# guptakhil/show-tell

Measured on AMD Instinct MI355X. Metric: training images/sec (ResNet101+GRU, emb=512, bs=128) at 1/2/4/8 MI355X, higher is better.
Workload: dtype bf16; 1 GPU; BASELINE configs[1]: ResNet-101 (train-mode BN, frozen) + 5-layer GRU decoder, E=H=512, V=10000, fwd+bwd+SGD step, synthetic COCO-shaped batch; batch_per_gpu=128, global_batch=128, image=3x224x224, parallelism=dp1

## Files before the change

### include/showtell_hip.h

```cpp
#ifndef SHOWTELL_HIP_H
#define SHOWTELL_HIP_H

#include <stddef.h>
#include <stdint.h>

#ifdef __cplusplus
extern "C" {
#endif

#define ST_F32 0
#define ST_BF16 1

#define ST_CELL_GRU 0
#define ST_CELL_LSTM 1

const char* st_last_error(void);
int st_version(void);

typedef struct {
  const void* x;
  const void* w;
  void* y;
  const float* bias;
  const float* scale;
// ... 24 lines not shown
} st_conv3x3_img_desc;
int st_conv3x3_img_supported(int H, int W, int C, int N);
int st_conv3x3_img(const st_conv3x3_img_desc* d, void* stream);
int st_conv3x3_s2_supported(int C, int N);
int st_conv3x3_s2(const st_conv3x3_img_desc* d, void* stream);
typedef struct {
  const void* x; const void* w_frag; void* y; const void* residual;
  float* stats; int stats_replicas;
  const float* scale; const float* shift; int relu;
  const float* in_stats; const float* in_gamma; const float* in_beta; float in_count; float in_eps; int in_stats_replicas;
  int B, Hin, Win, C, N, stride;
} st_conv1x1_wreg_desc;
int st_conv1x1_wreg_supported(int C, int N);
int st_conv1x1_wreg(const st_conv1x1_wreg_desc* d, void* stream);
int st_conv1x1_kstream_supported(int C, int N);
int st_conv1x1_kstream(const st_conv1x1_wreg_desc* d, void* stream);
typedef struct {
  const void* raw; const void* identity; void* x_out; const void* w_frag; void* y;
  float* stats; int stats_replicas;
  const float* f_stats; const float* f_gamma; const float* f_beta; float f_count; float f_eps; int f_stats_replicas;
  long rows; int C, N;
  const float* id_stats; const float* id_gamma; const float* id_beta; int id_stats_replicas;
} st_conv1x1_kfuse_desc;
int st_conv1x1_kfuse_supported(int C, int N);
int st_conv1x1_kfuse(const st_conv1x1_kfuse_desc* d, void* stream);
#ifdef ST_EXPERIMENTAL
int st_conv1x1_kfuse8(const st_conv1x1_kfuse_desc* d, void* stream);
#endif
typedef struct {
  const void* raw2; const void* w3_frag; const void* identity; void* x_out; const void* w1_frag; void* y;
  float* stats; int stats_replicas;
  const float* bn2_stats; const float* bn2_gamma; const float* bn2_beta; int bn2_replicas;
  const float* bn3_stats; const float* bn3_gamma; const float* bn3_beta; int bn3_replicas;
  const float* id_stats; const float* id_gamma; const float* id_beta; int id_replicas;
  float count; float eps;
  long rows; int C1, C2, N;
} st_conv_b2b_desc;
int st_conv_b2b_supported(int C1, int C2, int N);
int st_conv_b2b(const st_conv_b2b_desc* d, void* stream);
typedef struct {
  const void* x2; const void* w3_frag; const void* identity; void* x_out; const void* w1_frag; void* y;
  float* stats; int stats_replicas;
  const float* bn2_stats; const float* bn2_gamma; const float* bn2_beta; int bn2_replicas;
  const float* bn3_stats; const float* bn3_gamma; const float* bn3_beta; int bn3_replicas;
  float count; float eps;
  const float* scale3; const float* shift3; const float* scale1; const float* shift1; int relu1;
  long rows; int C1, C2, N;
  const float* id_stats; const float* id_gamma; const float* id_beta; int id_replicas;
} st_conv_c3c1_desc;
int st_conv_c3c1_supported(int C1, int C2, int N);
int st_conv_c3c1(const st_conv_c3c1_desc* d, void* stream);
int st_conv1x1_astat_supported(int C, int N);
int st_conv1x1_astat(const st_conv1x1_wreg_desc* d, void* stream);

int st_pack_conv_weight_frag(const float* w, void* out, int Cout, int Cin, int KH, int KW, int ntw, void* stream);

int st_tune(int reserved, int kc, int w8);
int st_prof_enable(int on);
int st_debug_stamps(unsigned long long* buf);
int st_prof_collect(double* ms, double* flops, long* launches);

typedef struct {
  const void* x; void* y; const void* res;
  const float* stats;  const float* gamma; const float* beta;
  const float* running_mean; const float* running_var;
  const float* res_stats; const float* res_gamma; const float* res_beta;
  const float* res_running_mean; const float* res_running_var;
  int res_bn;
  int dtype; long rows; int C; float count; float eps; int relu;
  int stats_replicas, res_stats_replicas;
} st_bn_act_desc;

int st_bn_act(const st_bn_act_desc* d, void* stream);

int st_bn_update_running(const float* stats, float* running_mean, float* running_var,
                         int C, float count, float momentum, void* stream);

int st_nchw_to_nhwc(const float* x, void* y, int dtype, int B, int C, int H, int W, int Cpad, void* stream);
int st_nchw_to_s2d16(const float* x, void* y, int dtype, int B, int H, int W, void* stream);
int st_stem_weight_s2d(const void* w, void* out, int dtype, int Cpad, void* stream);
int st_nhwc_to_ncp_f32(const void* x, float* y, int dtype, int B, int HW, int C, void* stream);
int st_maxpool3x3s2(const void* x, void* y, int dtype, int B, int H, int W, int C, void* stream);
int st_maxpool3x3s2_bn(const void* x, void* y, int dtype, int B, int H, int W, int C,
                       const float* stats, const float* gamma, const float* beta,
                       const float* running_mean, const float* running_var, float count, float eps, void* stream);
typedef struct {
  const void* x_s2d; const void* w_frag; void* y;
  float* stats; int stats_replicas;
  const float* gamma;
  const float* scale; const float* shift;
  int B, H, W;
} st_stem_conv_pool_desc;
int st_stem_conv_pool(const st_stem_conv_pool_desc* d, void* stream);
int st_stem_weight_frag(const void* w_s2d, void* out, void* stream);
int st_stem_weight_frag_packed(const void* w_packed, int Cpad, void* out, void* stream);
int st_global_avgpool(const void* x, void* y, int dtype, int out_dtype, int B, int HW, int C, void* stream);

typedef struct st_image_batch_desc {
  const uint8_t* src;
  int64_t src_bytes;
  const int64_t* offset;
  const int32_t* height;
  const int32_t* width;
  const int32_t* flip;
  int batch;
  int max_height, max_width;
// ... 161 lines not shown
```

### show-tell_amd/_lib.py

```python
import ctypes as C
import os

_HERE = os.path.dirname(os.path.abspath(__file__))
LIB_PATH = os.path.join(_HERE, "lib", "libshowtell_hip.so")

ST_F32, ST_BF16 = 0, 1
ST_CELL_GRU, ST_CELL_LSTM = 0, 1

c_p, c_i, c_f, c_l = C.c_void_p, C.c_int, C.c_float, C.c_long


class ConvDesc(C.Structure):
    _fields_ = [("x", c_p), ("w", c_p), ("y", c_p), ("bias", c_p), ("scale", c_p), ("shift", c_p),
                ("residual", c_p), ("stats", c_p), ("dtype", c_i), ("out_dtype", c_i),
                ("B", c_i), ("Hin", c_i), ("Win", c_i), ("Cin", c_i), ("Ho", c_i), ("Wo", c_i), ("N", c_i),
                ("KH", c_i), ("KW", c_i), ("stride", c_i), ("pad", c_i),
                ("ldx", c_i), ("ldw", c_i), ("ldy", c_i), ("relu", c_i), ("accumulate", c_i), ("Cin_logical", c_i), ("k_order", c_i), ("stats_replicas", c_i),
                ("in_stats", c_p), ("in_gamma", c_p), ("in_beta", c_p), ("in_count", c_f), ("in_eps", c_f), ("split_k", c_i)]


class Conv3x3ImgDesc(C.Structure):
    _fields_ = [("x", c_p), ("w_frag", c_p), ("y", c_p), ("stats", c_p), ("stats_replicas", c_i), ("scale", c_p), ("shift", c_p),
                ("relu", c_i), ("in_stats", c_p), ("in_gamma", c_p), ("in_beta", c_p), ("in_count", c_f), ("in_eps", c_f),
                ("B", c_i), ("H", c_i), ("W", c_i), ("C", c_i), ("N", c_i), ("in_stats_replicas", c_i)]
# ... 49 lines not shown


class RnnParams(C.Structure):
    _fields_ = [("cell", c_i), ("dtype", c_i), ("L", c_i), ("in0", c_i), ("H", c_i), ("V", c_i), ("E", c_i),
                ("emb", c_p), ("w_ih", c_p * ST_MAX_LAYERS), ("w_hh", c_p * ST_MAX_LAYERS),
                ("b_ih", c_p * ST_MAX_LAYERS), ("b_hh", c_p * ST_MAX_LAYERS), ("w_lin", c_p), ("b_lin", c_p)]


class RnnGrads(C.Structure):
    _fields_ = [("emb", c_p), ("w_ih", c_p * ST_MAX_LAYERS), ("w_hh", c_p * ST_MAX_LAYERS),
                ("b_ih", c_p * ST_MAX_LAYERS), ("b_hh", c_p * ST_MAX_LAYERS), ("w_lin", c_p), ("b_lin", c_p)]


class AttnParams(C.Structure):
    _fields_ = [("rnn", RnnParams), ("F", c_i), ("A", c_i), ("P", c_i),
                ("w_enc", c_p), ("b_enc", c_p), ("w_dec", c_p), ("b_dec", c_p), ("w_full", c_p), ("b_full", c_p),
                ("w_init_h", c_p), ("b_init_h", c_p), ("w_init_c", c_p), ("b_init_c", c_p), ("w_embed", c_p), ("b_embed", c_p)]


class AttnGrads(C.Structure):
    _fields_ = [("rnn", RnnGrads)] + [(n, c_p) for n in ("w_enc", "b_enc", "w_dec", "b_dec", "w_full", "b_full", "w_init_h", "b_init_h",
                                                        "w_init_c", "b_init_c", "w_embed", "b_embed")]


class PackedSeq(C.Structure):
    _fields_ = [("B", c_i), ("T", c_i), ("ntok", c_i), ("Tcap", c_i), ("batch_sizes_host", C.POINTER(c_i)),
                ("rows_b", c_p), ("rows_t", c_p), ("prev_row", c_p), ("caption", c_p)]


class ImageBatchDesc(C.Structure):
    _fields_ = [("src", c_p), ("src_bytes", C.c_int64), ("offset", c_p), ("height", c_p), ("width", c_p), ("flip", c_p), ("batch", c_i),
                ("max_height", c_i), ("max_width", c_i), ("out_h", c_i), ("out_w", c_i), ("lut", c_p), ("tmp", c_p),
                ("out", c_p), ("out_u8", c_p)]


_SIGS = {
    "st_version": ([], c_i),
    "st_image_transform": ([C.POINTER(ImageBatchDesc), c_p], c_i),
    "st_conv": ([C.POINTER(ConvDesc), c_p], c_i),
    "st_conv_batch": ([C.POINTER(ConvDesc), c_i, c_p], c_i),
    "st_conv3x3_img_supported": ([c_i, c_i, c_i, c_i], c_i),
    "st_conv3x3_img": ([C.POINTER(Conv3x3ImgDesc), c_p], c_i),
    "st_conv3x3_s2_supported": ([c_i, c_i], c_i),
    "st_conv3x3_s2": ([C.POINTER(Conv3x3ImgDesc), c_p], c_i),
    "st_conv1x1_wreg_supported": ([c_i, c_i], c_i),
    "st_conv1x1_wreg": ([C.POINTER(Conv1x1WregDesc), c_p], c_i),
    "st_conv1x1_kfuse": ([C.POINTER(Conv1x1KfuseDesc), c_p], c_i),
    "st_conv1x1_kfuse_supported": ([c_i, c_i], c_i),
    "st_conv1x1_kfuse8": ([C.POINTER(Conv1x1KfuseDesc), c_p], c_i),
    "st_conv_b2b": ([C.POINTER(ConvB2bDesc), c_p], c_i),
    "st_conv_b2b_supported": ([c_i, c_i, c_i], c_i),
    "st_conv1x1_astat_supported": ([c_i, c_i], c_i),
    "st_conv1x1_astat": ([C.POINTER(Conv1x1WregDesc), c_p], c_i),
    "st_conv1x1_kstream_supported": ([c_i, c_i], c_i),
    "st_conv1x1_kstream": ([C.POINTER(Conv1x1WregDesc), c_p], c_i),
    "st_pack_conv_weight_frag": ([c_p, c_p, c_i, c_i, c_i, c_i, c_i, c_p], c_i),
    "st_tune": ([c_i, c_i, c_i], c_i),
    "st_prof_enable": ([c_i], c_i),
    "st_debug_stamps": ([c_p], c_i),
    "st_prof_collect": ([C.POINTER(C.c_double), C.POINTER(C.c_double), C.POINTER(c_l)], c_i),
    "st_bn_act": ([C.POINTER(BnActDesc), c_p], c_i),
    "st_bn_update_running": ([c_p, c_p, c_p, c_i, c_f, c_f, c_p], c_i),
    "st_nchw_to_nhwc": ([c_p, c_p, c_i, c_i, c_i, c_i, c_i, c_i, c_p], c_i),
    "st_nchw_to_s2d16": ([c_p, c_p, c_i, c_i, c_i, c_i, c_p], c_i),
    "st_stem_weight_s2d": ([c_p, c_p, c_i, c_i, c_p], c_i),
    "st_stem_weight_frag": ([c_p, c_p, c_p], c_i),
    "st_stem_weight_frag_packed": ([c_p, c_i, c_p, c_p], c_i),
    "st_stem_conv_pool": ([C.POINTER(StemConvPoolDesc), c_p], c_i),
    "st_nhwc_to_ncp_f32": ([c_p, c_p, c_i, c_i, c_i, c_i, c_p], c_i),
    "st_maxpool3x3s2": ([c_p, c_p, c_i, c_i, c_i, c_i, c_i, c_p], c_i),
    "st_maxpool3x3s2_bn": ([c_p, c_p, c_i, c_i, c_i, c_i, c_i, c_p, c_p, c_p, c_p, c_p, c_f, c_f, c_p], c_i),
    "st_global_avgpool": ([c_p, c_p, c_i, c_i, c_i, c_i, c_i, c_p], c_i),
    "st_cast": ([c_p, c_p, c_i, c_i, c_l, c_p], c_i),
    "st_transpose": ([c_p, c_p, c_i, c_i, c_i, c_i, c_i, c_p], c_i),
    "st_transpose_colsum": ([c_p, c_p, c_p, c_i, c_i, c_i, c_i, c_i, c_p], c_i),
    "st_transpose_batch": ([c_p, c_p, c_p, c_i, c_i, c_i, c_i, c_i, c_i, c_p, c_p, c_p], c_i),
    "st_pack_conv_weight": ([c_p, c_p, c_i, c_i, c_i, c_i, c_i, c_i, c_i, c_p], c_i),
    "st_cast2d": ([c_p, c_p, c_i, c_i, c_i, c_i, c_i, c_i, c_p], c_i),
    "st_rnn_vocab_ld": ([c_i], c_i),
    "st_rnn_workspace_bytes": ([C.POINTER(RnnParams), C.POINTER(PackedSeq)], C.c_size_t),
    "st_rnn_forward": ([C.POINTER(RnnParams), C.POINTER(PackedSeq), c_p, c_p, c_p, C.c_size_t, c_p, c_i, c_i, c_p, c_i, c_p], c_i),
    "st_rnn_fused_loss_supported": ([C.POINTER(RnnParams)], c_i),
    "st_rnn_fused_loss_bytes": ([C.POINTER(RnnParams), C.POINTER(PackedSeq)], C.c_size_t),
    "st_rnn_fused_loss": ([C.POINTER(RnnParams), C.POINTER(PackedSeq), c_p, C.c_size_t, c_p, c_p, C.c_size_t, c_p, c_p], c_i),
    "st_rnn_fused_dlogits": ([C.POINTER(RnnParams), C.POINTER(PackedSeq), c_p, C.c_size_t, c_p, c_p, c_p, c_p, c_i, c_p], c_i),
    "st_rnn_backward": ([C.POINTER(RnnParams), C.POINTER(RnnGrads), C.POINTER(PackedSeq), c_p, c_p, c_i, c_p, c_p, C.c_size_t,
                         c_p, c_p, c_p], c_i),
    "st_rnn_greedy_workspace_bytes": ([C.POINTER(RnnParams), c_i], C.c_size_t),
    "st_rnn_greedy": ([C.POINTER(RnnParams), c_p, c_i, c_i, c_p, C.c_size_t, c_p, c_p, c_p], c_i),
    "st_rnn_greedy_last_route": ([], c_i),
    "st_rnn_step": ([C.POINTER(RnnParams), c_p, c_i, c_p, c_p, c_p, c_p, c_p, c_i, c_p], c_i),
    "st_embedding_rows": ([c_p, c_p, c_p, c_i, c_i, c_i, c_i, c_i, c_p], c_i),
    "st_gather_state": ([c_p, c_p, c_p, c_i, c_i, c_i, c_i, c_i, c_p], c_i),
    "st_softmax_topk": ([c_p, c_i, c_i, c_i, c_i, c_p, c_p, c_i, c_p], c_i),
    "st_beam_select": ([c_p, c_p, c_p, c_p, c_p, c_i, c_i, c_i, c_l, c_p, c_p, c_p, c_p, c_p, c_p], c_i),
    "st_sample_rows": ([c_p, c_i, c_i, c_i, c_p, c_i, c_f, c_i, c_l, c_p, c_p, c_p, c_i, c_i, c_p, c_p], c_i),
    "st_rnn_sample_workspace_bytes": ([C.POINTER(RnnParams), c_i], C.c_size_t),
    "st_rnn_sample": ([C.POINTER(RnnParams), c_p, c_i, c_i, c_p, c_f, c_i, c_l, c_p, C.c_size_t, c_p, c_p, c_p], c_i),
    "st_attn_workspace_bytes": ([c_p, c_p], C.c_size_t),
    "st_attn_forward": ([c_p, c_p, c_p, c_p, c_p, C.c_size_t, c_p, c_i, c_i, c_p, c_i, c_p], c_i),
    "st_attn_backward": ([c_p, c_p, c_p, c_p, c_p, c_i, c_p, c_p, c_f, c_p, c_p, C.c_size_t, c_p], c_i),
    "st_attn_reg_loss": ([c_p, c_i, c_i, c_i, c_f, c_p, c_p], c_i),
    "st_attn_greedy_workspace_bytes": ([c_p, c_i], C.c_size_t),
    "st_attn_greedy": ([c_p, c_p, c_i, c_i, c_l, c_p, C.c_size_t, c_p, c_p], c_i),
    "st_attn_greedy_alphas": ([c_p, c_p, c_i, c_i, c_l, c_p, C.c_size_t, c_p, c_p, c_p], c_i),
    "st_attn_sample_workspace_bytes": ([c_p, c_i], C.c_size_t),
# ... 66 lines not shown
```

### show-tell_amd/csrc/resnet.cpp

```cpp
#include "common.h"
#include <vector>
#include <map>
#include <mutex>
#include <new>
#include <string>
#include <string.h>
#include <stdlib.h>

struct ConvL { int cin, cout, k, stride, pad; size_t woff; size_t bnoff; int korder; size_t woff_frag; int ntw; };
struct BlockL { int c1, c2, c3, ds; int stride; };
static inline bool use_astat(const ConvL& c) {
  if (c.k != 1) return false;
  if (c.stride == 1) return (c.cin == 256 && c.cout == 1024) || (c.cin == 512 && c.cout == 2048);
  return c.stride == 2 && ((c.cin == 256 && c.cout == 512) || (c.cin == 512 && c.cout == 1024));
}

struct BnTable { int n; int end[160]; float count[160]; int soff[160]; int rep[160]; };
struct PendingUpdate { BnTable tab; const float* stats; };

struct st_resnet {
  int version, dtype, bottleneck, cpad0;
  std::vector<ConvL> convs;
  std::vector<BlockL> blocks;
  size_t wtotal = 0, bntotal = 0;
// ... 116 lines not shown
        b.c2 = add(planes[li], planes[li], 3, s, 1);
        b.c3 = add(planes[li], planes[li] * 4, 1, 1, 0);
      } else {
        b.c1 = add(inpl, planes[li], 3, s, 1);
        b.c2 = add(planes[li], planes[li], 3, 1, 1);
      }
      if (bi == 0 && (s != 1 || inpl != planes[li] * exp)) b.ds = add(inpl, planes[li] * exp, 1, s, 0);
      inpl = planes[li] * exp;
      r->blocks.push_back(b);
    }
  r->feat_dim = inpl;
  ST_CHECK(r->convs.size() <= 160, "st_resnet_create: too many layers");
  *out = r;
  return 0;
}

extern "C" void st_resnet_destroy(st_resnet* r) { delete r; }
extern "C" int st_resnet_num_convs(const st_resnet* r) { return r ? (int)r->convs.size() : -1; }
extern "C" int st_resnet_feat_dim(const st_resnet* r) { return r ? r->feat_dim : -1; }
extern "C" size_t st_resnet_weight_elems(const st_resnet* r) { return r ? r->wtotal : 0; }
extern "C" size_t st_resnet_bn_channels(const st_resnet* r) { return r ? r->bntotal : 0; }

extern "C" int st_resnet_conv_info(const st_resnet* r, int i, int* cin, int* cout, int* k, int* stride, int* pad,
                                   int* cin_padded, size_t* weight_offset, size_t* bn_offset, int* k_order,
                                   size_t* frag_weight_offset, int* frag_ntw) {
  ST_CHECK(r && i >= 0 && i < (int)r->convs.size(), "st_resnet_conv_info: bad index %d", i);
  const ConvL& c = r->convs[i];
  if (cin) *cin = c.cin;
  if (cout) *cout = c.cout;
  if (k) *k = c.k;
  if (stride) *stride = c.stride;
  if (pad) *pad = c.pad;
  if (cin_padded) *cin_padded = c.cin == 3 ? r->cpad0 : c.cin;
  if (weight_offset) *weight_offset = c.woff;
  if (bn_offset) *bn_offset = c.bnoff;
  if (k_order) *k_order = c.korder;
  if (frag_weight_offset) *frag_weight_offset = c.woff_frag;
  if (frag_ntw) *frag_ntw = c.ntw;
  return 0;
}

extern "C" int st_resnet_set_taps(st_resnet* r, void* buf, size_t bytes) {
  ST_CHECK(r && (buf || bytes == 0), "st_resnet_set_taps: null pointer");
  std::lock_guard<std::mutex> lk(r->mu);
  r->taps = buf; r->taps_bytes = buf ? bytes : 0;
  return 0;
}

namespace {
FILE* layer_log() {
  static FILE* f = [] { const char* e = getenv("ST_LAYER_LOG"); return e && *e ? fopen(e, "w") : nullptr; }();
  return f;
}
struct Layout { size_t in_bytes, s2dw_bytes, stem_bytes, wide_bytes, narrow_bytes, stats_bytes, fold_bytes, total; };
inline bool stem_s2d(int H, int W) { return H % 2 == 0 && W % 2 == 0; }
Layout make_layout(const st_resnet* r, int B, int H, int W) {
  const size_t es = st_dtype_size(r->dtype);
  Layout p;
  p.in_bytes = align256((size_t)B * H * W * r->cpad0 * es);
  if (stem_s2d(H, W)) { const size_t b2 = align256((size_t)B * (H / 2 + 3) * (W / 2 + 3) * 16 * es); if (b2 > p.in_bytes) p.in_bytes = b2; }
  p.s2dw_bytes = align256((size_t)64 * 256 * es);
  const int h1 = conv_out(H, 7, 2, 3), w1 = conv_out(W, 7, 2, 3);
  p.stem_bytes = align256((size_t)B * h1 * w1 * 64 * es);
  const int h2 = conv_out(h1, 3, 2, 1), w2 = conv_out(w1, 3, 2, 1);
  const size_t wide_c = r->bottleneck ? 256 : 64;
  p.wide_bytes = align256((size_t)B * h2 * w2 * wide_c * es);
  p.narrow_bytes = align256((size_t)B * h2 * w2 * 128 * es);
  p.stats_bytes = align256((2 * r->bntotal + (size_t)kStatsRepFloats * r->convs.size()) * sizeof(float));
  p.fold_bytes = align256(2 * r->bntotal * sizeof(float));
  p.total = p.in_bytes + p.s2dw_bytes + p.stem_bytes + 3 * p.wide_bytes + 2 * p.narrow_bytes + p.stats_bytes + p.fold_bytes;
  return p;
}

enum Route {
  R_IGEMM, R_IMG, R_S2, R_WREG, R_ASTAT, R_KSTREAM,
  R_KFUSE, R_B2B, R_B2B0, R_C3C1,
  R_STEM, R_STEM_POOL, R_MAXPOOL,
  R_BN_ACT, R_REDUCE, R_TAP
};
enum Slot { S_NONE = -1, S_IN, S_STEM, S_WIDE, S_NARROW = S_WIDE + 3, S_COUNT = S_NARROW + 2 };

struct Launch {
  Route route;
  int ci;
  int hin, win;
  int x, y, res, xout;
  int relu;
  int in_ci;
  int pc;
  int id_ci;
  int rep_out, rep_in;
};
constexpr int kMaxLaunches = 768;
struct FwdPlan { int n; bool s2d; int h, w, out; BnTable tab; Launch l[kMaxLaunches]; };

int plan_forward(const st_resnet* r, int B, int H, int W, bool train, FwdPlan& p) {
  const int nconv = (int)r->convs.size(), nblk = (int)r->blocks.size();
  ST_CHECK(nconv <= 160 && 8 + 14 * nblk <= kMaxLaunches, "st_resnet_forward: too many layers");
  const bool bf16 = r->dtype == ST_BF16;
  BnTable& tab = p.tab;
  tab.n = nconv;
  for (int i = 0; i < nconv; ++i) { tab.end[i] = (int)(r->convs[i].bnoff + r->convs[i].cout); tab.count[i] = 1.f; tab.soff[i] = 0; tab.rep[i] = 1; }
  int hin[160], win[160], hout[160], wout[160];
  Route rt[160];
  auto geo = [&](int ci, int h, int w, bool res) {
    const ConvL& c = r->convs[ci];
    hin[ci] = h; win[ci] = w;
    hout[ci] = conv_out(h, c.k, c.stride, c.pad); wout[ci] = conv_out(w, c.k, c.stride, c.pad);
    tab.count[ci] = (float)((long)B * hout[ci] * wout[ci]);
    rt[ci] = R_IGEMM;
    if (!bf16 || c.ntw == 0) return;
    if (c.k == 1 && (!res || (c.stride == 1 && c.cin <= 512))) rt[ci] = use_astat(c) ? R_ASTAT : c.cin > 512 ? R_KSTREAM : R_WREG;
    else if (c.k == 3 && c.stride == 1 && !res && st_conv3x3_img_supported(h, w, c.cin, c.cout) == c.ntw) rt[ci] = R_IMG;
    else if (c.k == 3 && c.stride == 2 && !res && st_conv3x3_s2_supported(c.cin, c.cout) == c.ntw && (long)B * h * w * c.cin * 2 < (1L << 31))
      rt[ci] = R_S2;
  };
  geo(0, H, W, false);
  rt[0] = R_STEM;
  int h = conv_out(hout[0], 3, 2, 1), w = conv_out(wout[0], 3, 2, 1);
  for (const BlockL& b : r->blocks) {
    geo(b.c1, h, w, false);
    if (b.ds >= 0) geo(b.ds, h, w, false);
    if (r->bottleneck) { geo(b.c2, hout[b.c1], wout[b.c1], false); geo(b.c3, hout[b.c2], wout[b.c2], !train); }
// ... 159 lines not shown
    case R_BN_ACT:
      fam = "bn_act"; what = l.res != S_NONE ? "bn + identity + relu" : "bn + relu"; cin = c.cout; k = stride = hin = win = 0;
      by = rows * c.cout * (l.res != S_NONE ? 3.0 : 2.0) * es; break;
    case R_REDUCE:
      fam = "bn_reduce_replicas"; what = "statistics replicas -> replica 0"; cin = c.cout; k = stride = hin = win = 0; break;
    default: return 0;
  }
  return snprintf(buf, n, "%s,%s,%d,%d,%d,%d,%d,%d,%.0f,%.0f,%d,%d\n", fam, what, cin, cout, k, stride, hin, win, fl, by, l.rep_out, l.rep_in);
}
}

extern "C" size_t st_resnet_workspace_bytes(const st_resnet* r, int B, int H, int W) {
  if (!r || B <= 0 || H < 32 || W < 32) return 0;
  return make_layout(r, B, H, W).total;
}

extern "C" int st_resnet_plan(const st_resnet* r, int B, int H, int W, int train, char* buf, size_t bytes) {
  if (!r || B <= 0 || H < 32 || W < 32) { st_set_error("st_resnet_plan: bad arguments"); return -1; }
  FwdPlan p;
  if (plan_forward(r, B, H, W, train != 0, p)) return -1;
  std::string text;
  char line[256];
  for (int i = 0; i < p.n; ++i) text.append(line, format_launch(r, B, p.l[i], line, sizeof(line)));
  if (buf && bytes > text.size()) memcpy(buf, text.c_str(), text.size() + 1);
  return (int)text.size();
}

extern "C" int st_resnet_forward(const st_resnet* r, const float* images_nchw, int B, int H, int W,
                                 const void* weights, const float* bn_gamma, const float* bn_beta,
                                 float* bn_running_mean, float* bn_running_var,
                                 int train, float momentum, float eps,
                                 void* workspace, size_t workspace_bytes,
                                 void* feat_nhwc_out, void* pooled_out, int pooled_dtype, float* ncp_out,
                                 void* stream) {
  ST_CHECK(r && images_nchw && weights && bn_gamma && bn_beta && bn_running_mean && bn_running_var && workspace,
           "st_resnet_forward: null pointer");
  ST_CHECK(B > 0 && H >= 32 && W >= 32, "st_resnet_forward: bad input size %dx%dx%d", B, H, W);
  const Layout lay = make_layout(r, B, H, W);
  ST_CHECK(workspace_bytes >= lay.total, "st_resnet_forward: workspace too small (%zu < %zu)", workspace_bytes, lay.total);
  FwdPlan p;
  if (plan_forward(r, B, H, W, train != 0, p)) return 1;
  const BnTable& tab = p.tab;
  hipStream_t st = reinterpret_cast<hipStream_t>(stream);
  const int dt = r->dtype;
  const size_t es = st_dtype_size(dt);
  char* ws = reinterpret_cast<char*>(workspace);
  char* slot[S_COUNT];
  slot[S_IN] = ws; ws += lay.in_bytes;
  char* s2dw = ws; ws += lay.s2dw_bytes;
  slot[S_STEM] = ws; ws += lay.stem_bytes;
  for (int i = 0; i < 3; ++i) { slot[S_WIDE + i] = ws; ws += lay.wide_bytes; }
  for (int i = 0; i < 2; ++i) { slot[S_NARROW + i] = ws; ws += lay.narrow_bytes; }
  float* stats = reinterpret_cast<float*>(ws); ws += lay.stats_bytes;
  float* fold = reinterpret_cast<float*>(ws);
  const int total = (int)r->bntotal;
  float* fscale = fold; float* fshift = fold + total;

  if (train) {
    if (hipMemsetAsync(stats, 0, lay.stats_bytes, st) != hipSuccess) { st_set_error("memset failed"); return 1; }
  } else {
    hipLaunchKernelGGL(bn_fold_kernel, dim3((total + 255) / 256), dim3(256), 0, st, bn_gamma, bn_beta, bn_running_mean,
                       bn_running_var, fscale, fshift, total, eps);
    ST_LAUNCH_CHECK();
  }
  if (p.s2d) {
    if (st_nchw_to_s2d16(images_nchw, slot[S_IN], dt, B, H, W, stream)) return 1;
  } else if (st_nchw_to_nhwc(images_nchw, slot[S_IN], dt, B, 3, H, W, r->cpad0, stream)) return 1;

  auto S = [&](int s) -> void* { return s == S_NONE ? nullptr : slot[s]; };
  auto wts = [&](size_t off) { return reinterpret_cast<const char*>(weights) + off * es; };
  struct BnRef { const float* stats; const float* gamma; const float* beta; int rep; };
  auto bn = [&](int ci) { const ConvL& c = r->convs[ci]; return BnRef{stats + tab.soff[ci], bn_gamma + c.bnoff, bn_beta + c.bnoff, tab.rep[ci]}; };
  auto set_in = [&](auto& d, const Launch& l) {
    if (l.in_ci < 0) return;
    const BnRef b = bn(l.in_ci);
    d.in_stats = b.stats; d.in_gamma = b.gamma; d.in_beta = b.beta; d.in_count = tab.count[l.in_ci]; d.in_eps = eps;
  };
  auto set_out = [&](auto& d, const Launch& l) {
    const ConvL& c = r->convs[l.ci];
    if (train) { d.stats = stats + tab.soff[l.ci]; d.stats_replicas = l.rep_out; }
    else { d.scale = fscale + c.bnoff; d.shift = fshift + c.bnoff; d.relu = l.relu; }
  };
  auto set_fused = [&](auto& k, const Launch& l) {
    const BnRef b2 = bn(l.in_ci), b3 = bn(l.pc);
    k.bn2_stats = b2.stats; k.bn2_gamma = b2.gamma; k.bn2_beta = b2.beta; k.bn2_replicas = b2.rep;
    k.bn3_stats = b3.stats; k.bn3_gamma = b3.gamma; k.bn3_beta = b3.beta; k.bn3_replicas = b3.rep;
    if (l.id_ci >= 0) { const BnRef i = bn(l.id_ci); k.id_stats = i.stats; k.id_gamma = i.gamma; k.id_beta = i.beta; k.id_replicas = i.rep; }
    k.count = tab.count[l.pc]; k.eps = eps;
  };
  size_t taps_used = 0;
  auto run = [&](const Launch& l) -> int {
    const ConvL& c = r->convs[l.ci];
    const long rows = (long)B * l.hin * l.win;
    switch (l.route) {
      case R_STEM: case R_IGEMM: {
        st_conv_desc d{};
        const int cin_p = c.cin == 3 ? r->cpad0 : c.cin;
        d.x = S(l.x); d.w = wts(c.woff); d.y = S(l.y); d.residual = S(l.res);
        d.dtype = dt; d.out_dtype = dt;
        d.B = B; d.Hin = l.hin; d.Win = l.win; d.Cin = cin_p;
        d.Ho = conv_out(l.hin, c.k, c.stride, c.pad); d.Wo = conv_out(l.win, c.k, c.stride, c.pad);
        d.N = c.cout; d.KH = c.k; d.KW = c.k; d.stride = c.stride; d.pad = c.pad;
        d.ldx = cin_p; d.ldw = c.k * c.k * cin_p; d.ldy = c.cout; d.Cin_logical = c.cin; d.k_order = c.korder;
        if (l.route == R_STEM && p.s2d) {
          if (st_stem_weight_s2d(wts(c.woff), s2dw, dt, r->cpad0, stream)) return 1;
          d.w = s2dw; d.Hin = l.hin / 2 + 3; d.Win = l.win / 2 + 3; d.Cin = 64; d.ldx = 16; d.KH = 4; d.KW = 1; d.stride = 1; d.pad = 0;
          d.ldw = 256; d.Cin_logical = 36;
        }
        set_in(d, l); set_out(d, l);
        return st_conv(&d, stream);
      }
      case R_IMG: case R_S2: {
        st_conv3x3_img_desc g{};
        g.x = S(l.x); g.w_frag = wts(c.woff_frag); g.y = S(l.y);
        g.B = B; g.H = l.hin; g.W = l.win; g.C = c.cin; g.N = c.cout; g.in_stats_replicas = l.rep_in;
        set_in(g, l); set_out(g, l);
        return l.route == R_IMG ? st_conv3x3_img(&g, stream) : st_conv3x3_s2(&g, stream);
      }
      case R_WREG: case R_ASTAT: case R_KSTREAM: {
        st_conv1x1_wreg_desc g{};
        g.x = S(l.x); g.w_frag = wts(c.woff_frag); g.y = S(l.y); g.residual = S(l.res);
        g.B = B; g.Hin = l.hin; g.Win = l.win; g.C = c.cin; g.N = c.cout; g.stride = c.stride; g.in_stats_replicas = l.rep_in;
        set_in(g, l); set_out(g, l);
        if (l.route == R_WREG) return st_conv1x1_wreg(&g, stream);
        if (l.route == R_ASTAT) return st_conv1x1_astat(&g, stream);
        ST_CHECK(!g.in_stats, "st_resnet_forward: the long-K pointwise kernel has no input transform");
        return st_conv1x1_kstream(&g, stream);
      }
      case R_KFUSE: {
        st_conv1x1_kfuse_desc k{};
        const BnRef f = bn(l.pc);
        k.raw = S(l.x); k.identity = S(l.res); k.x_out = S(l.xout); k.w_frag = wts(c.woff_frag); k.y = S(l.y);
        k.stats = stats + tab.soff[l.ci]; k.stats_replicas = l.rep_out;
        k.f_stats = f.stats; k.f_gamma = f.gamma; k.f_beta = f.beta; k.f_count = tab.count[l.pc]; k.f_eps = eps; k.f_stats_replicas = f.rep;
        k.rows = rows; k.C = c.cin; k.N = c.cout;
        if (l.id_ci >= 0) { const BnRef i = bn(l.id_ci); k.id_stats = i.stats; k.id_gamma = i.gamma; k.id_beta = i.beta; k.id_stats_replicas = i.rep; }
        return st_conv1x1_kfuse(&k, stream);
      }
      case R_B2B: case R_B2B0: {
        const ConvL& c3 = r->convs[l.pc];
        st_conv_b2b_desc k{};
        k.raw2 = S(l.x); k.w3_frag = wts(c3.woff_frag); k.identity = S(l.res); k.x_out = S(l.xout);
        set_fused(k, l);
        k.rows = rows; k.C1 = c3.cin; k.C2 = c3.cout;
        if (l.route == R_B2B) {
          k.w1_frag = wts(c.woff_frag); k.y = S(l.y); k.stats = stats + tab.soff[l.ci]; k.stats_replicas = l.rep_out; k.N = c.cout;
        }
        return st_conv_b2b(&k, stream);
      }
      case R_C3C1: {
        const ConvL& c3 = r->convs[l.pc];
        st_conv_c3c1_desc k{};
        k.x2 = S(l.x); k.w3_frag = wts(c3.woff_frag); k.identity = S(l.res); k.x_out = S(l.xout); k.w1_frag = wts(c.woff_frag); k.y = S(l.y);
        if (train) {
          k.stats = stats + tab.soff[l.ci]; k.stats_replicas = l.rep_out;
          set_fused(k, l);
        } else {
          k.scale3 = fscale + c3.bnoff; k.shift3 = fshift + c3.bnoff; k.scale1 = fscale + c.bnoff; k.shift1 = fshift + c.bnoff; k.relu1 = l.relu;
        }
        k.rows = rows; k.C1 = c3.cin; k.C2 = c3.cout; k.N = c.cout;
        return st_conv_c3c1(&k, stream);
      }
      case R_STEM_POOL: {
        if (st_stem_weight_frag_packed(wts(c.woff), r->cpad0, slot[S_STEM], stream)) return 1;
        st_stem_conv_pool_desc sd{};
        sd.x_s2d = S(l.x); sd.w_frag = slot[S_STEM]; sd.y = S(l.y); sd.B = B; sd.H = l.hin; sd.W = l.win;
        if (train) { sd.stats = stats + tab.soff[l.ci]; sd.stats_replicas = l.rep_out; sd.gamma = bn_gamma + c.bnoff; }
        else { sd.scale = fscale + c.bnoff; sd.shift = fshift + c.bnoff; }
        return st_stem_conv_pool(&sd, stream);
      }
      case R_MAXPOOL:
        if (l.in_ci < 0) return st_maxpool3x3s2(S(l.x), S(l.y), dt, B, l.hin, l.win, c.cout, stream);
        return st_maxpool3x3s2_bn(S(l.x), S(l.y), dt, B, l.hin, l.win, c.cout, stats + tab.soff[l.ci], bn_gamma + c.bnoff, bn_beta + c.bnoff,
                                  nullptr, nullptr, tab.count[l.ci], eps, stream);
      case R_BN_ACT: {
        st_bn_act_desc d{};
// ... 67 lines not shown
```

Baseline: 30990 images/sec.

## Compute 1x1 conv BN statistics via input Gram matrix instead of full output

Adds a Gram-matrix path for stats-only 1x1 convolutions. Per-channel mean and variance of the conv output are derived as W·sum(x) and diag(W·XᵀX·Wᵀ), so the K×N output GEMM is replaced by a K×K Gram GEMM plus a small finish kernel. It is enabled by default only for C=64, the first-stage expansion conv, and selectable for other widths by environment variable. It needs extra scratch workspace and an additional kernel launch with atomics, and it changes the summation order of the statistics.

```diff
diff --git a/include/showtell_hip.h b/include/showtell_hip.h
--- a/include/showtell_hip.h
+++ b/include/showtell_hip.h
@@ -100,6 +100,9 @@
 int st_conv_c3c1(const st_conv_c3c1_desc* d, void* stream);
 int st_conv1x1_astat_supported(int C, int N);
 int st_conv1x1_astat(const st_conv1x1_wreg_desc* d, void* stream);
+int st_conv1x1_gram_stats_supported(int C, int N);
+size_t st_conv1x1_gram_stats_scratch_bytes(int C, long rows);
+int st_conv1x1_gram_stats(const st_conv1x1_wreg_desc* d, void* scratch, size_t scratch_bytes, void* stream);
 
 int st_pack_conv_weight_frag(const float* w, void* out, int Cout, int Cin, int KH, int KW, int ntw, void* stream);
 
diff --git a/show-tell_amd/_lib.py b/show-tell_amd/_lib.py
--- a/show-tell_amd/_lib.py
+++ b/show-tell_amd/_lib.py
@@ -125,6 +125,9 @@
     "st_conv_b2b_supported": ([c_i, c_i, c_i], c_i),
     "st_conv1x1_astat_supported": ([c_i, c_i], c_i),
     "st_conv1x1_astat": ([C.POINTER(Conv1x1WregDesc), c_p], c_i),
+    "st_conv1x1_gram_stats_supported": ([c_i, c_i], c_i),
+    "st_conv1x1_gram_stats_scratch_bytes": ([c_i, c_l], C.c_size_t),
+    "st_conv1x1_gram_stats": ([C.POINTER(Conv1x1WregDesc), c_p, C.c_size_t, c_p], c_i),
     "st_conv1x1_kstream_supported": ([c_i, c_i], c_i),
     "st_conv1x1_kstream": ([C.POINTER(Conv1x1WregDesc), c_p], c_i),
     "st_pack_conv_weight_frag": ([c_p, c_p, c_i, c_i, c_i, c_i, c_i, c_p], c_i),
diff --git a/show-tell_amd/csrc/conv_gram.hip b/show-tell_amd/csrc/conv_gram.hip
--- /dev/null
+++ b/show-tell_amd/csrc/conv_gram.hip
@@ -0,0 +1,290 @@
+#include "common.h"
+#include "prof.h"
+#include <stdlib.h>
+#include <string.h>
+
+namespace {
+
+typedef __attribute__((ext_vector_type(4))) short s16x4;
+typedef __attribute__((ext_vector_type(2))) float f32x2;
+
+struct GramArgs {
+  const bf16_t* x; const bf16_t* w;
+  float* stats; int srep;
+  const float* in_stats; const float* in_gamma; const float* in_beta; float in_count, in_eps; int in_srep;
+  float* part;
+  int M, N, nstage, spw, P;
+};
+
+__device__ __forceinline__ void bn_relu_chunk_g(u32x4& v, const float* sc, const float* sh) {
+#pragma unroll
+  for (int d = 0; d < 4; ++d) {
+    const float lo = fmaxf(__uint_as_float(v[d] << 16) * sc[2 * d] + sh[2 * d], 0.f);
+    const float hi = fmaxf(__uint_as_float(v[d] & 0xffff0000u) * sc[2 * d + 1] + sh[2 * d + 1], 0.f);
+    v[d] = pack_bf16x2(lo, hi);
+  }
+}
+
+__device__ __forceinline__ f32x4 mfma_bf16_g(const u32x4& a, const u32x4& b, const f32x4& c) {
+  return __builtin_amdgcn_mfma_f32_16x16x32_bf16(*reinterpret_cast<const bf16x8*>(&a), *reinterpret_cast<const bf16x8*>(&b), c, 0, 0, 0);
+}
+
+__device__ __forceinline__ u32x2 lds_tr16(const char* p) {
+  const s16x4 v = __builtin_amdgcn_ds_read_tr16_b64_v4i16((__attribute__((address_space(3))) s16x4*)(p));
+  return *reinterpret_cast<const u32x2*>(&v);
+}
+
+constexpr int kGramStageBytes = 16384;
+
+template <int K, int NT>
+__global__ __launch_bounds__(NT) __attribute__((amdgpu_waves_per_eu(NT / 256, NT / 256))) void gram_partial_kernel(GramArgs a) {
+  constexpr int PIX = 2 * K + 32, BM = kGramStageBytes / K, CH8 = K / 8, RPP = NT / CH8, NL = BM / RPP;
+  constexpr int TR = K / 64, TC = K / 16, KB = BM / 32;
+  constexpr int CG = NT / 256, TCW = TC / CG;
+  constexpr int TCH = TCW < 8 ? TCW : 8;
+  static_assert(NL * NT == 2048 && BM % 32 == 0 && TCW % TCH == 0, "stage shape");
+  extern __shared__ __attribute__((aligned(16))) char smem[];
+  float* coef = reinterpret_cast<float*>(smem + 2 * BM * PIX);
+
+  const int tid = threadIdx.x, lane = tid & 63;
+  const int wid = __builtin_amdgcn_readfirstlane(tid >> 6);
+  const int rg = wid & 3, cg = wid >> 2;
+  const int s0 = blockIdx.x * a.spw;
+  const int s1 = s0 + a.spw < a.nstage ? s0 + a.spw : a.nstage;
+  const bool xf = a.in_stats != nullptr;
+  StatHead shd;
+  if (xf) stat_head_issue(shd, a.in_stats, a.in_srep, K, tid % K, a.in_gamma, a.in_beta);
+
+  const int cch = tid % CH8, lrow = tid / CH8;
+  u32x4 v[NL];
+  auto load = [&](int s) {
+#pragma unroll
+    for (int i = 0; i < NL; ++i) {
+      int m = s * BM + lrow + i * RPP;
+      m = m < a.M ? m : a.M - 1;
+      v[i] = *reinterpret_cast<const u32x4*>(a.x + (size_t)m * K + cch * 8);
+    }
+  };
+  load(s0);
+  float sc[8], sh[8];
+  if (xf) {
+    if (tid < K) stat_head_finish(shd, a.in_stats, a.in_srep, K, tid, 1.0f / a.in_count, a.in_eps, coef[tid], coef[K + tid]);
+    __syncthreads();
+#pragma unroll
+    for (int e = 0; e < 8; ++e) { sc[e] = coef[cch * 8 + e]; sh[e] = coef[K + cch * 8 + e]; }
+  }
+
+  const int r16 = lane & 15, g4 = lane >> 4;
+  const int frag0 = (4 * (4 * (g4 >> 1) + (g4 & 1)) + (r16 >> 2)) * PIX + 8 * (r16 & 3);
+  auto frag = [&](const char* buf, int kb, int t) {
+    const char* p = buf + frag0 + kb * 32 * PIX + t * 32;
+    const u32x2 lo = lds_tr16(p), hi = lds_tr16(p + 8 * PIX);
+    return u32x4{lo[0], lo[1], hi[0], hi[1]};
+  };
+
+  f32x4 acc[TR][TCW];
+#pragma unroll
+  for (int i = 0; i < TR; ++i)
+#pragma unroll
+    for (int t = 0; t < TCW; ++t) acc[i][t] = f32x4{0.f, 0.f, 0.f, 0.f};
+  float cs[8];
+#pragma unroll
+  for (int e = 0; e < 8; ++e) cs[e] = 0.f;
+
+  for (int s = s0; s < s1; ++s) {
+    char* buf = smem + ((s - s0) & 1) * BM * PIX;
+#pragma unroll
+    for (int i = 0; i < NL; ++i) {
+      if (xf) bn_relu_chunk_g(v[i], sc, sh);
+      if (s * BM + lrow + i * RPP >= a.M) v[i] = u32x4{0u, 0u, 0u, 0u};
+      *reinterpret_cast<u32x4*>(buf + (lrow + i * RPP) * PIX + cch * 16) = v[i];
+#pragma unroll
+      for (int d = 0; d < 4; ++d) { cs[2 * d] += __uint_as_float(v[i][d] << 16); cs[2 * d + 1] += __uint_as_float(v[i][d] & 0xffff0000u); }
+    }
+    if (s + 1 < s1) load(s + 1);
+    __syncthreads();
+#pragma unroll
+    for (int kb = 0; kb < KB; ++kb) {
+      u32x4 fa[TR];
+#pragma unroll
+      for (int i = 0; i < TR; ++i) fa[i] = frag(buf, kb, TR * rg + i);
+#pragma unroll
+      for (int t0 = 0; t0 < TCW; t0 += TCH) {
+        u32x4 fb[TCH];
+#pragma unroll
+        for (int t = 0; t < TCH; ++t) fb[t] = frag(buf, kb, cg * TCW + t0 + t);
+#pragma unroll
+        for (int i = 0; i < TR; ++i)
+#pragma unroll
+          for (int t = 0; t < TCH; ++t) acc[i][t0 + t] = mfma_bf16_g(fa[i], fb[t], acc[i][t0 + t]);
+      }
+    }
+  }
+
+  float* gp = a.part + (size_t)blockIdx.x * (K * K + K);
+#pragma unroll
+  for (int i = 0; i < TR; ++i) {
+    const int c0 = 16 * (TR * rg + i) + 4 * g4;
+#pragma unroll
+    for (int t = 0; t < TCW; ++t) *reinterpret_cast<f32x4*>(gp + (size_t)(16 * (cg * TCW + t) + r16) * K + c0) = acc[i][t];
+  }
+  float* sred = reinterpret_cast<float*>(smem);
+  __syncthreads();
+#pragma unroll
+  for (int e = 0; e < 8; e += 4) *reinterpret_cast<f32x4*>(sred + lrow * K + cch * 8 + e) = f32x4{cs[e], cs[e + 1], cs[e + 2], cs[e + 3]};
+  __syncthreads();
+  if (tid < K) {
+    float sm = 0.f;
+#pragma unroll
+    for (int q = 0; q < RPP; ++q) sm += sred[q * K + tid];
+    gp[K * K + tid] = sm;
+  }
+}
+
+template <int K, int CPT, int CS>
+__global__ __launch_bounds__(256) void gram_finish_kernel(GramArgs a) {
+  constexpr int JB = 4, KS = K / 32, GR = 256 / K, PS = K * K + K;
+  static_assert(K == 64 || K == 128 || K == 256, "one float4 of the four rows per thread and partial group");
+  __shared__ __attribute__((aligned(16))) float sred[GR * JB * K];
+  __shared__ __attribute__((aligned(16))) float sgt[K * JB];
+  __shared__ __attribute__((aligned(16))) float ssum[4][JB];
+
+  const int tid = threadIdx.x, lane = tid & 63, wid = tid >> 6;
+  const int J0 = blockIdx.x * JB;
+  {
+    const int vq = tid % K, gq = tid / K;
+    const float* src = a.part + (size_t)J0 * K + vq * 4;
+    f32x4 sum{0.f, 0.f, 0.f, 0.f};
+#pragma unroll 16
+    for (int p = gq; p < a.P; p += GR) sum += *reinterpret_cast<const f32x4*>(src + (size_t)p * PS);
+    *reinterpret_cast<f32x4*>(sred + (gq * K + vq) * 4) = sum;
+    f32x4 sv{0.f, 0.f, 0.f, 0.f};
+    for (int p = tid; p < a.P; p += 256) sv += *reinterpret_cast<const f32x4*>(a.part + (size_t)p * PS + K * K + J0);
+#pragma unroll
+    for (int e = 0; e < JB; ++e) sv[e] = wave_sum(sv[e]);
+    if (lane == 0) *reinterpret_cast<f32x4*>(&ssum[wid][0]) = sv;
+    __syncthreads();
+    if (gq == 0) {
+#pragma unroll
+      for (int g = 1; g < GR; ++g) sum += *reinterpret_cast<const f32x4*>(sred + (g * K + vq) * 4);
+      const int j = vq / (K / 4), i0 = 4 * (vq % (K / 4));
+#pragma unroll
+      for (int e = 0; e < 4; ++e) sgt[(i0 + e) * JB + j] = sum[e];
+    }
+    __syncthreads();
+  }
+
+  const int r = tid & 15, T0 = (tid >> 4) + 16 * CPT * blockIdx.y;
+  const u32x4* wl = reinterpret_cast<const u32x4*>(a.w);
+  f32x2 t[CPT][2];
+#pragma unroll
+  for (int u = 0; u < CPT; ++u) { t[u][0] = f32x2{0.f, 0.f}; t[u][1] = f32x2{0.f, 0.f}; }
+#pragma unroll 8
+  for (int kq = 0; kq < K / 8; ++kq) {
+    u32x4 wv[CPT];
+#pragma unroll
+    for (int u = 0; u < CPT; ++u) wv[u] = wl[((size_t)(T0 + 16 * u) * KS + (kq >> 2)) * 64 + (kq & 3) * 16 + r];
+#pragma unroll
+    for (int e = 0; e < 8; ++e) {
+      const f32x4 gv = *reinterpret_cast<const f32x4*>(sgt + (kq * 8 + e) * JB);
+      const f32x2 g01{gv[0], gv[1]}, g23{gv[2], gv[3]};
+#pragma unroll
+      for (int u = 0; u < CPT; ++u) {
+        const uint32_t d = wv[u][e >> 1];
+        const float wf = __uint_as_float((e & 1) ? (d & 0xffff0000u) : (d << 16));
+        const f32x2 w2{wf, wf};
+        t[u][0] = w2 * g01 + t[u][0];
+        t[u][1] = w2 * g23 + t[u][1];
+      }
+    }
+  }
+  float sj[JB];
+#pragma unroll
+  for (int e = 0; e < JB; ++e) sj[e] = ssum[0][e] + ssum[1][e] + ssum[2][e] + ssum[3][e];
+  float* sdst = a.stats + (a.srep > 1 ? (size_t)((blockIdx.x + blockIdx.y) % a.srep) * 2 * a.N : 0);
+  const uint16_t* w16 = reinterpret_cast<const uint16_t*>(a.w);
+#pragma unroll
+  for (int u = 0; u < CPT; ++u) {
+    const int T = T0 + 16 * u;
+    const u32x2 wj = *reinterpret_cast<const u32x2*>(w16 + (((size_t)T * KS + J0 / 32) * 64 + ((J0 % 32) / 8) * 16 + r) * 8 + J0 % 8);
+    const float w0 = __uint_as_float(wj[0] << 16), w1 = __uint_as_float(wj[0] & 0xffff0000u);
+    const float w2 = __uint_as_float(wj[1] << 16), w3 = __uint_as_float(wj[1] & 0xffff0000u);
+    const float sq = t[u][0][0] * w0 + t[u][0][1] * w1 + t[u][1][0] * w2 + t[u][1][1] * w3;
+    const float sm = w0 * sj[0] + w1 * sj[1] + w2 * sj[2] + w3 * sj[3];
+    const int c = (T >> 1) * 32 + 8 * (r >> 2) + 4 * (T & 1) + (r & 3);
+    atomicAdd(sdst + c, sm);
+    atomicAdd(sdst + a.N + c, sq);
+  }
+}
+
+inline int gram_partials(int K, long M, int* spw_out) {
+  const int BM = kGramStageBytes / K;
+  const long nstage = (M + BM - 1) / BM;
+  const int target = K == 256 ? 64 : K == 128 ? 128 : 256;
+  long spw = (nstage + target - 1) / target;
+  if (spw < 1) spw = 1;
+  if (spw_out) *spw_out = (int)spw;
+  return (int)((nstage + spw - 1) / spw);
+}
+
+template <int K, int NT, int CPT, int CS>
+int launch_gram(GramArgs& a, hipStream_t st) {
+  constexpr int BM = kGramStageBytes / K;
+  constexpr int lds = 2 * BM * (2 * K + 32) + 2 * K * (int)sizeof(float);
+  static int attr_set[64] = {};
+  int dev = 0;
+  (void)hipGetDevice(&dev);
+  if (dev >= 0 && dev < 64 && !attr_set[dev]) {
+    (void)hipFuncSetAttribute(reinterpret_cast<const void*>(&gram_partial_kernel<K, NT>), hipFuncAttributeMaxDynamicSharedMemorySize, lds);
+    attr_set[dev] = 1;
+  }
+  hipLaunchKernelGGL((gram_partial_kernel<K, NT>), dim3(a.P), dim3(NT), lds, st, a);
+  hipLaunchKernelGGL((gram_finish_kernel<K, CPT, CS>), dim3(K / 4, CS), dim3(256), 0, st, a);
+  return 0;
+}
+}
+
+extern "C" int st_conv1x1_gram_stats_supported(int C, int N) {
+  if (C == 64 && N == 256) return st_conv1x1_wreg_supported(C, N) == 2;
+  if (C == 128 && N == 512) return st_conv1x1_wreg_supported(C, N) == 2;
+  if (C == 256 && N == 1024) return st_conv1x1_astat_supported(C, N) == 2;
+  return 0;
+}
+
+extern "C" size_t st_conv1x1_gram_stats_scratch_bytes(int C, long rows) {
+  if (rows <= 0 || (C != 64 && C != 128 && C != 256)) return 0;
+  return (size_t)gram_partials(C, rows, nullptr) * ((size_t)C * C + C) * sizeof(float);
+}
+
+extern "C" int st_conv1x1_gram_stats(const st_conv1x1_wreg_desc* d, void* scratch, size_t scratch_bytes, void* stream) {
+  ST_CHECK(d && d->x && d->w_frag && d->stats && scratch, "st_conv1x1_gram_stats: null pointer");
+  ST_CHECK(!d->y && !d->residual && !d->scale && !d->shift && !d->relu, "st_conv1x1_gram_stats: statistics only (no output, no epilogue)");
+  ST_CHECK(st_conv1x1_gram_stats_supported(d->C, d->N), "st_conv1x1_gram_stats: unsupported geometry C=%d N=%d", d->C, d->N);
+  ST_CHECK(d->B > 0 && d->Hin > 0 && d->Win > 0 && d->stride == 1, "st_conv1x1_gram_stats: bad geometry (stride 1 only)");
+  ST_CHECK(!d->in_stats || (d->in_gamma && d->in_beta && d->in_count > 0.f), "st_conv1x1_gram_stats: input transform needs gamma, beta, count");
+  ST_CHECK(d->stats_replicas >= 0 && d->stats_replicas <= 1024 && d->in_stats_replicas >= 0 && d->in_stats_replicas <= 1024, "st_conv1x1_gram_stats: bad stats_replicas");
+  const long M = (long)d->B * d->Hin * d->Win;
+  ST_CHECK(M < (1L << 31) - 4096, "st_conv1x1_gram_stats: too many rows");
+  ST_CHECK(scratch_bytes >= st_conv1x1_gram_stats_scratch_bytes(d->C, M), "st_conv1x1_gram_stats: scratch too small (%zu < %zu)", scratch_bytes,
+           st_conv1x1_gram_stats_scratch_bytes(d->C, M));
+  ST_CHECK((reinterpret_cast<uintptr_t>(scratch) & 15) == 0, "st_conv1x1_gram_stats: scratch must be 16-byte aligned");
+  GramArgs a{};
+  a.x = reinterpret_cast<const bf16_t*>(d->x); a.w = reinterpret_cast<const bf16_t*>(d->w_frag);
+  a.stats = d->stats; a.srep = d->stats_replicas;
+  a.in_stats = d->in_stats; a.in_gamma = d->in_gamma; a.in_beta = d->in_beta; a.in_count = d->in_count; a.in_eps = d->in_eps;
+  a.in_srep = d->in_stats_replicas > 1 ? d->in_stats_replicas : 1;
+  a.part = reinterpret_cast<float*>(scratch);
+  a.M = (int)M; a.N = d->N;
+  const int BM = kGramStageBytes / d->C;
+  a.nstage = (int)((M + BM - 1) / BM);
+  a.P = gram_partials(d->C, M, &a.spw);
+  hipStream_t st = reinterpret_cast<hipStream_t>(stream);
+  const double flops = 2.0 * (double)a.nstage * BM * d->C * (d->C + 16) + 2.0 * (double)d->N * d->C * (d->C + 1);
+  StProfScope prof(d->C == 64 ? 12 : d->C == 128 ? 13 : 18, flops, st);
+  if (d->C == 64) launch_gram<64, 256, 1, 1>(a, st);
+  else if (d->C == 128) launch_gram<128, 256, 1, 2>(a, st);
+  else launch_gram<256, 512, 2, 2>(a, st);
+  prof.end(st);
+  ST_LAUNCH_CHECK();
+  return 0;
+}
diff --git a/show-tell_amd/csrc/resnet.cpp b/show-tell_amd/csrc/resnet.cpp
--- a/show-tell_amd/csrc/resnet.cpp
+++ b/show-tell_amd/csrc/resnet.cpp
@@ -192,7 +192,20 @@
   static FILE* f = [] { const char* e = getenv("ST_LAYER_LOG"); return e && *e ? fopen(e, "w") : nullptr; }();
   return f;
 }
-struct Layout { size_t in_bytes, s2dw_bytes, stem_bytes, wide_bytes, narrow_bytes, stats_bytes, fold_bytes, total; };
+bool gram_stats_on(int K) {
+  const char* e = getenv("ST_GRAM_STATS");
+  if (!e || !*e) return K == 64;
+  for (const char* p = e; *p;) {
+    char* end = nullptr;
+    const long v = strtol(p, &end, 10);
+    if (end == p) break;
+    if (v == K && v != 0) return true;
+    p = *end == ',' ? end + 1 : end;
+    if (*end && *end != ',') break;
+  }
+  return false;
+}
+struct Layout { size_t in_bytes, s2dw_bytes, stem_bytes, wide_bytes, narrow_bytes, stats_bytes, fold_bytes, gram_bytes, total; };
 inline bool stem_s2d(int H, int W) { return H % 2 == 0 && W % 2 == 0; }
 Layout make_layout(const st_resnet* r, int B, int H, int W) {
   const size_t es = st_dtype_size(r->dtype);
@@ -208,7 +221,18 @@
   p.narrow_bytes = align256((size_t)B * h2 * w2 * 128 * es);
   p.stats_bytes = align256((2 * r->bntotal + (size_t)kStatsRepFloats * r->convs.size()) * sizeof(float));
   p.fold_bytes = align256(2 * r->bntotal * sizeof(float));
-  p.total = p.in_bytes + p.s2dw_bytes + p.stem_bytes + 3 * p.wide_bytes + 2 * p.narrow_bytes + p.stats_bytes + p.fold_bytes;
+  p.gram_bytes = 0;
+  if (r->bottleneck && r->dtype == ST_BF16) {
+    int h = h2, w = w2;
+    for (const BlockL& b : r->blocks) {
+      h = (h - 1) / b.stride + 1; w = (w - 1) / b.stride + 1;
+      const ConvL& c3 = r->convs[b.c3];
+      if (!st_conv1x1_gram_stats_supported(c3.cin, c3.cout)) continue;
+      const size_t g = align256(st_conv1x1_gram_stats_scratch_bytes(c3.cin, (long)B * h * w));
+      if (g > p.gram_bytes) p.gram_bytes = g;
+    }
+  }
+  p.total = p.in_bytes + p.s2dw_bytes + p.stem_bytes + 3 * p.wide_bytes + 2 * p.narrow_bytes + p.stats_bytes + p.fold_bytes + p.gram_bytes;
   return p;
 }
 
@@ -474,7 +498,8 @@
   for (int i = 0; i < 3; ++i) { slot[S_WIDE + i] = ws; ws += lay.wide_bytes; }
   for (int i = 0; i < 2; ++i) { slot[S_NARROW + i] = ws; ws += lay.narrow_bytes; }
   float* stats = reinterpret_cast<float*>(ws); ws += lay.stats_bytes;
-  float* fold = reinterpret_cast<float*>(ws);
+  float* fold = reinterpret_cast<float*>(ws); ws += lay.fold_bytes;
+  void* gram = ws;
   const int total = (int)r->bntotal;
   float* fscale = fold; float* fshift = fold + total;
 
@@ -544,6 +569,9 @@
         g.x = S(l.x); g.w_frag = wts(c.woff_frag); g.y = S(l.y); g.residual = S(l.res);
         g.B = B; g.Hin = l.hin; g.Win = l.win; g.C = c.cin; g.N = c.cout; g.stride = c.stride; g.in_stats_replicas = l.rep_in;
         set_in(g, l); set_out(g, l);
+        if (train && dt == ST_BF16 && l.y == S_NONE && l.res == S_NONE && c.stride == 1 && gram_stats_on(c.cin) &&
+            st_conv1x1_gram_stats_supported(c.cin, c.cout))
+          return st_conv1x1_gram_stats(&g, gram, lay.gram_bytes, stream);
         if (l.route == R_WREG) return st_conv1x1_wreg(&g, stream);
         if (l.route == R_ASTAT) return st_conv1x1_astat(&g, stream);
         ST_CHECK(!g.in_stats, "st_resnet_forward: the long-K pointwise kernel has no input transform");
```

Result: no change. 31230 images/sec, median of 6 (+0.8%).
